# francescovidaich964/TensorNetworkForML

Measured on AMD Instinct MI355X. Metric: sweep-steps/sec, 28x28 MNIST-shaped, bond=20, batch=5000 per GPU, higher is better.
Workload: dtype f32; 1 GPU; c3: N=784 sites, D=2, L=2, bond 20, batch 5000/GPU, softmax+full_cross_ent, trunc=fixed, L2_flag=True; pass = hand-over of one of 4 staged batches + forward + 783-step sweep; global_batch=5000, sweep_steps_per_pass=783, parallelism=dp1, distinct_batches=4

## Files before the change

### tensornetworkforml_amd/csrc/kernels_narrow.hip

```cpp
#include "tnml_internal.h"
#include "jacobi_device.h"
#include "small_gemm_device.h"
#include "wide_pipe_device.h"

namespace tnml {

__device__ inline double wave_sum_f64(double v) {
  v += dpp_f64<0xB1>(v);
  v += dpp_f64<0x4E>(v);
  v += dpp_f64<0x141>(v);
  v += dpp_f64<0x140>(v);
  const double r0 = wave_read_f64(v, 0), r1 = wave_read_f64(v, 16), r2 = wave_read_f64(v, 32), r3 = wave_read_f64(v, 48);
  return (r0 + r1) + (r2 + r3);
}

template <int BUF>
__device__ inline void block_sum3(double &a, double &b, double &c, double *scratch) {
  const int lane = threadIdx.x & 63, wave = threadIdx.x >> 6, nw = blockDim.x >> 6;
  double *s = scratch + BUF * 64;
  a = wave_sum_f64(a); b = wave_sum_f64(b); c = wave_sum_f64(c);
  if (lane == 0) { s[wave] = a; s[16 + wave] = b; s[32 + wave] = c; }
  lds_barrier();
  const int w = lane & 15;
  double ta = w < nw ? s[w] : 0.0, tb = w < nw ? s[16 + w] : 0.0, tc = w < nw ? s[32 + w] : 0.0;
// ... 203 lines not shown
  const int r = D * h, c = D * g * L;
  const bool short_rows = (r <= c);
  const int n = short_rows ? r : c, ne = n + (n & 1), len = short_rows ? c : r;

  unsigned long long t_c0 = 0, t_r0 = 0, t_c1 = 0, t_c2 = 0, t_c2b = 0, t_c2c = 0;
  unsigned long long t_p[5] = {0, 0, 0, 0, 0};
#define TNML_STAMP(i) if (p.stamps && tid == 0) t_p[i] = __builtin_amdgcn_s_memtime()
  if (p.stamps && tid == 0) { t_c0 = __builtin_amdgcn_s_memtime(); t_r0 = __builtin_amdgcn_s_memrealtime(); }
  const int RWz = kD * kD * p.g * p.L;
  const bool fast0 = p.pipe && !p.persist && (size_t)p.z_rows * RWz + (size_t)p.z_rows * h <= (size_t)((float *)k.sOrd - k.fBp) &&
                     Bs <= 8 * NT && p.z_rows * RWz <= 16 * NT && p.z_rows * h <= 4 * NT && h * h <= 2 * NT && g * g <= 2 * NT;
  const PersistLds PL = persist_lds(smem_raw + p.persist_off, p.Mcap);
  float *sRaw = k.fBp;
  if (p.persist) {
    if (tid == 0) {
      const int bad = spin_wait_ge(p.pready, p.pwant, p.abort_flag, 1);
      if (bad == 1) { atomicOr(p.status, 4); __hip_atomic_store(p.abort_flag, 1u, __ATOMIC_RELAXED, __HIP_MEMORY_SCOPE_AGENT); }
      k.sFlag[3] = bad;
    }
    lds_barrier();
    if (k.sFlag[3]) return true;
    if (p.stamps && tid == 0) { p.stamps[20] = (double)(__builtin_amdgcn_s_memtime() - t_c0); p.stamps[28] = (double)(t_r0 & ((1ull << 40) - 1)); p.stamps[29] = (double)(__builtin_amdgcn_s_memrealtime() & ((1ull << 40) - 1)); }
    if (tid < kMetricSlots) k.sTail[tid] = ld_sc1(p.zred + p.zsize + tid);
    for (int e = tid; e < h * h; e += NT) k.dNh[e] = p.Nh ? PL.Nh[e] : 1.0;
    const __amdgpu_buffer_rsrc_t rR = sc1_rsrc(p.prepRaw), rB = sc1_rsrc(p.prepB), rG = sc1_rsrc(p.prepG);
    tn_uvec4 qr[2], qb[2], qg[4];
#pragma unroll
    for (int u = 0; u < 2; ++u) { const int e = 4 * (tid + u * NT); if (e < Bs) { qr[u] = ld_sc1_b128(rR, (unsigned)e * 4u); qb[u] = ld_sc1_b128(rB, (unsigned)e * 4u); } }
#pragma unroll
    for (int u = 0; u < 4; ++u) { const int e = 2 * (tid + u * NT); if (p.l2_flag && e < Bs) qg[u] = ld_sc1_b128(rG, (unsigned)e * 8u); }
#pragma unroll
    for (int u = 0; u < 2; ++u) { const int e = 4 * (tid + u * NT); if (e < Bs) { *reinterpret_cast<tn_uvec4 *>(sRaw + e) = qr[u]; *reinterpret_cast<tn_uvec4 *>(k.fB + e) = qb[u]; } }
#pragma unroll
    for (int u = 0; u < 4; ++u) { const int e = 2 * (tid + u * NT); if (p.l2_flag && e < Bs) *reinterpret_cast<tn_uvec4 *>(k.dG + e) = qg[u]; }
  }
  float *sZ = k.fBp, *sZc = sZ + (size_t)p.z_rows * RWz;
  if (fast0) {
    const int zr = p.z_rows, nz = p.z_first ? 0 : zr * RWz, nzc = p.z_first ? 0 : zr * h;
    const float *zc = p.zcore.base;
    float4 rz[4], rb[2];
    double2 rg[4];
    float rc[4];
    double rnh[2], rng[2];
#pragma unroll
    for (int u = 0; u < 4; ++u) { const int e = 4 * (tid + u * NT); rz[u] = e < nz ? *reinterpret_cast<const float4 *>(p.zred + e) : make_float4(0.f, 0.f, 0.f, 0.f); }
#pragma unroll
    for (int u = 0; u < 2; ++u) { const int e = 4 * (tid + u * NT); rb[u] = (p.prep_ready && e < Bs) ? *reinterpret_cast<const float4 *>(p.prepB + e) : make_float4(0.f, 0.f, 0.f, 0.f); }
#pragma unroll
    for (int u = 0; u < 4; ++u) { const int e = 2 * (tid + u * NT); rg[u] = (p.prep_ready && p.l2_flag && e < Bs) ? *reinterpret_cast<const double2 *>(p.prepG + e) : make_double2(0.0, 0.0); }
    const float inv_h = 1.0f / (float)h;
#pragma unroll
    for (int u = 0; u < 4; ++u) {
      const int e = tid + u * NT, i2 = (int)(((float)e + 0.5f) * inv_h), hh = e - i2 * h;
      rc[u] = e < nzc ? zc[(i2 >> 1) * p.zcore.s_in + (i2 & 1) * p.zcore.s_d + hh * p.zcore.s_out] : 0.f;
    }
#pragma unroll
    for (int u = 0; u < 2; ++u) {
      const int e = tid + u * NT;
      rnh[u] = (p.Nh && e < h * h) ? p.Nh[e] : 1.0;
      rng[u] = (p.Ng && e < g * g) ? p.Ng[e] : 1.0;
    }
#pragma unroll
    for (int u = 0; u < 4; ++u) { const int e = 4 * (tid + u * NT); if (e < nz) *reinterpret_cast<float4 *>(sZ + e) = rz[u]; }
#pragma unroll
    for (int u = 0; u < 2; ++u) { const int e = 4 * (tid + u * NT); if (p.prep_ready && e < Bs) *reinterpret_cast<float4 *>(k.fB + e) = rb[u]; }
#pragma unroll
    for (int u = 0; u < 4; ++u) { const int e = 2 * (tid + u * NT); if (p.prep_ready && p.l2_flag && e < Bs) *reinterpret_cast<double2 *>(k.dG + e) = rg[u]; }
// ... 85 lines not shown
      k.sLab[e] = p.lab.base[h_ * p.lab.s_in + d * p.lab.s_d + s_ * p.lab.s_out + l];
    }
    for (int e = tid; e < s * D * g; e += NT) {
      const int g_ = e % g, q = e / g;
      const int d = q % D, s_ = q / D;
      k.sPl[e] = p.pl.base[s_ * p.pl.s_in + d * p.pl.s_d + g_ * p.pl.s_out];
    }
  } else {
    for (int e = tid; e < Bs; e += NT) k.fB[e] = p.Bdirect[e];
  }
  if (!fast0 && !p.persist) {
    for (int e = tid; e < h * h; e += NT) k.dNh[e] = p.Nh ? p.Nh[e] : 1.0;
    for (int e = tid; e < g * g; e += NT) k.dNg[e] = p.Ng ? p.Ng[e] : 1.0;
  }
  lds_barrier();

  TNML_STAMP(0);
  const int RW = D * D * g * L;
  if (!p.Bdirect && !p.fused && !p.prep_ready && !p.persist) {
    const int QW = D * g;
    small_gemm_f64(L, h * D, QW, s,
                   [&](int l, int i, int kk) { return (double)k.sLab[(i * s + kk) * L + l]; },
                   [&](int l, int kk, int j) { return (double)k.sPl[kk * QW + j]; },
                   [&](int l, int i, int j, double v) { k.fB[(i * QW + j) * L + l] = (float)v; });
  }
  lds_barrier();

  TNML_STAMP(1);
  if (p.l2_flag && !p.fused && !p.prep_ready && !p.persist) {
    mm_lds(1, h, RW, h, k.dNh, 0, 1, h, k.fB, 0, RW, 1, [&](int, int i, int j, double v) { k.dT[i * RW + j] = v; });
    lds_barrier();
    mm_lds(L, Bs / (g * L), g, g, k.dT, 1, g * L, L, k.dNg, 0, g, 1,
           [&](int l, int i, int j, double v) { k.dG[(i * g + j) * L + l] = v; });
    lds_barrier();
  }
  TNML_STAMP(2);
  double sumB = 0.0, sumD = 0.0, l2 = 0.0;
  constexpr int kMaxPer = 8;
  float redv[kMaxPer];
#pragma unroll
  for (int u = 0; u < kMaxPer; ++u) {
    const int e = tid + u * NT;
    redv[u] = (e < Bs && !p.persist && !(p.pipe && !p.z_first)) ? ldred(e) : 0.f;
  }
#pragma unroll
  for (int u = 0; u < kMaxPer; ++u) {
    const int e = tid + u * NT;
    if (e >= Bs) break;
    const double bv = (double)k.fB[e];
    const double raw = p.persist ? (double)sRaw[e] : ((p.pipe && !p.z_first) ? k.dT[e] : (double)redv[u]);
    double wdterm;
    if (p.l2_flag) {
      const double gv = k.dG[e];
      l2 += bv * gv;
      wdterm = 2.0 * (double)p.wd * gv;
    } else {
      wdterm = (double)p.wd * bv;
    }
    const double dv = raw - wdterm;
    if (p.dbg) {
      p.dbg[e] = bv;
      p.dbg[Bs + e] = raw;
      p.dbg[3 * (size_t)Bs + e] = wdterm;
    }
    k.dG[e] = dv;
    sumB += fabs(bv);
// ... 503 lines not shown
           [&](int dk, int h_, int sp, double acc) {
             const float v = (float)acc;
             k.sCb[__mul24(h_ * D + dk, mk) + sp] = v;
             if (p.persist) PL.Ad[__mul24(h_ * D + dk, mk) + sp] = acc;
             st_behind(__mul24(h_, ob_s_h) + dk * ob_s_d + __mul24(sp, ob_s_m), v);
           });
  }
  lds_barrier();
  if (p.persist) {
    if (wave_u == (NT >> 6) - 1) {
      const int ln = tid & 63;
      const __amdgpu_buffer_rsrc_t rP = sc1_rsrc(p.Apub);
      for (int e = ln; e < (r * mk) >> 1; e += 64) st_sc1_b128(rP, (unsigned)e * 16u, pack_d2(PL.Ad[2 * e], PL.Ad[2 * e + 1]));
      for (int e = ln; e < (mk + 1) >> 1; e += 64) {
        const double i0 = k.dSq[ne + 2 * e], i1 = 2 * e + 1 < mk ? k.dSq[ne + 2 * e + 1] : 0.0;
        st_sc1_b128(rP, (unsigned)(r * mk + 2 * e) * 8u, pack_d2(i0 * i0, i1 * i1));
      }
      asm volatile("s_waitcnt vmcnt(0)" ::: "memory");
      if (ln == 0) { unsigned *const aflag = p.aflag; __hip_atomic_store(aflag, (unsigned)p.coretoken, __ATOMIC_RELAXED, __HIP_MEMORY_SCOPE_AGENT); }
    }
  }

  if (p.stamps && tid == 0) t_c2c = __builtin_amdgcn_s_memtime();
  if (Nh_new) {
    if (!short_rows) {
      mm_lds(1, h, DM, h, k.dNh, 0, h, 1, k.sCb, 0, DM, 1, store_T2);
      lds_barrier();
    }
    mm_lds(1, mk, mk, h * D, k.sCb, 0, 1, mk, k.dT2, 0, mk, 1,
           [&](int, int i, int j, double v) {
             Nh_new[__mul24(i, mk) + j] = v;
             if (p.persist) PL.Nh[__mul24(i, mk) + j] = v;
           });
    if (p.persist) {
      lds_barrier();
      const __amdgpu_buffer_rsrc_t rP = sc1_rsrc(p.Apub);
      const int oN = persist_pub_off(r * mk, mk), nn2 = mk * mk;
      for (int e = tid; e < (nn2 + 1) >> 1; e += NT)
        st_sc1_b128(rP, (unsigned)(oN + 2 * e) * 8u, pack_d2(PL.Nh[2 * e], 2 * e + 1 < nn2 ? PL.Nh[2 * e + 1] : 0.0));
    }
  }

  if (p.stamps && tid == 0) {
    const unsigned long long t_c3 = __builtin_amdgcn_s_memtime(), t_r3 = __builtin_amdgcn_s_memrealtime();
    p.stamps[0] = (double)(t_c1 - t_c0); p.stamps[1] = (double)(t_c2 - t_c1); p.stamps[2] = (double)(t_c3 - t_c2);
    p.stamps[3] = (double)(t_r3 - t_r0); p.stamps[4] = (double)sweeps; p.stamps[5] = (double)n;
    p.stamps[50] = (double)round_idx;
    for (int i = 0; i < 5; ++i) p.stamps[9 + i] = (double)(t_p[i] - (i ? t_p[i - 1] : t_c0));
    p.stamps[6] = (double)(t_c2b - t_c2); p.stamps[7] = (double)(t_c2c - t_c2b); p.stamps[8] = (double)(t_c3 - t_c2c);
  }

  if (tid == 0 && p.metrics) {
    const double cnt = (double)ldtail(3);
    const double inv = cnt > 0 ? 1.0 / cnt : 0.0;
    p.metrics[0] = (float)((double)ldtail(0) * inv);
    p.metrics[1] = (float)((double)ldtail(1) * inv / (double)L);
    if (ldtail(2) != 0.f) atomicOr(p.status, 1);
  }
  if (p.persist) {
    asm volatile("s_waitcnt vmcnt(0)" ::: "memory");
    lds_barrier();
    if (tid == 0) { unsigned *const coreflag = p.coreflag; __hip_atomic_store(coreflag, (unsigned)p.coretoken, __ATOMIC_RELAXED, __HIP_MEMORY_SCOPE_AGENT); }
  }
  if (p.done_flag) {
    asm volatile("s_waitcnt vmcnt(0)" ::: "memory");
    __syncthreads();
    if (wave_u == 0) {
      __builtin_amdgcn_fence(__ATOMIC_RELEASE, "agent");
      if (tid == 0) __hip_atomic_store(p.done_flag, p.done_val, __ATOMIC_RELAXED, __HIP_MEMORY_SCOPE_AGENT);
    }
  }
  return false;
}
// ... 84 lines not shown
        for (int e = tid; e < nW; e += NT) {
          const int l = e % L, q = e / L, s_ = q % s, d = r0 + q / s;
          sW[e] = t.lab.base[d * t.lab.s_d + s_ * t.lab.s_out + l];
        }
      }
      for (int e = tid; e < s * DG; e += NT) {
        const int g_ = e % g, q = e / g, d = q % D, s_ = q / D;
        sP[e] = t.pl.base[s_ * t.pl.s_in + d * t.pl.s_d + g_ * t.pl.s_out];
      }
      if (t.l2_flag) for (int e = tid; e < g * g; e += NT) sNg[e] = t.Ng ? t.Ng[e] : 1.0;
      lds_barrier();
      mm_lds(L, nr, DG, s, sW, 1, s * L, L, sP, 0, DG, 1, [&](int l, int row, int col, double v) { oT[(row * DG + col) * L + l] = v; });
      lds_barrier();
      if (t.l2_flag)
        mm_lds(L, nr * D, g, g, oT, 1, g * L, L, sNg, 0, g, 1, [&](int l, int i, int j, double v) { oN[(i * g + j) * L + l] = v; });
      const int nT = nr * DG * L;
      double *Tdst = t.T + (size_t)r0 * DG * L, *Ndst = t.TN + (size_t)r0 * DG * L;
      for (int e = tid; e < nT; e += NT) __hip_atomic_store(Tdst + e, oT[e], __ATOMIC_RELAXED, __HIP_MEMORY_SCOPE_AGENT);
      if (t.l2_flag) {
        lds_barrier();
        for (int e = tid; e < nT; e += NT) __hip_atomic_store(Ndst + e, oN[e], __ATOMIC_RELAXED, __HIP_MEMORY_SCOPE_AGENT);
      }
    }
    asm volatile("s_waitcnt vmcnt(0)" ::: "memory");
    lds_barrier();
    if (tid == 0) __hip_atomic_fetch_add(t.tcnt, 1u, __ATOMIC_RELAXED, __HIP_MEMORY_SCOPE_AGENT);
    return false;
  }
  const bool even_split = RW % nH == 0;
  const int cw = (RW + nH - 1) / nH, c0 = even_split ? hid * cw : min(RW, hid * cw), nc = even_split ? cw : min(RW, c0 + cw) - c0;
  const int cw2 = 2 * cw;
  double *sA = (double *)smem_raw;
  double *sIv = sA + (((size_t)zr * h + 1) & ~(size_t)1);
  double *sNh = sIv + ((h + 1) & ~1);
  double *sS = sNh + (((size_t)h * h + 1) & ~(size_t)1);
  float *sOut = (float *)(sS + persist_helper_ss_doubles(zr, h, cw));
  double *sP2 = (double *)sOut + (size_t)h * cw;
  float *sZf = (float *)(sP2 + (size_t)h * cw);
  float *sAff = sZf + (size_t)zr * cw;
  double *hst = (t.stamps && hid == 0 && tid == 0) ? t.stamps : nullptr;
  double *hst2 = (t.stamps && hid == 0) ? t.stamps : nullptr;
  auto rt = []() { return (double)(__builtin_amdgcn_s_memrealtime() & ((1ull << 40) - 1)); };
  if (tid == 0) { if (hst) hst[22] = rt(); give_up(spin_wait_ge(t.tcnt, (unsigned)nH, t.abort_flag)); if (hst) hst[30] = rt(); }
  lds_barrier();
  if (sBad) return true;
  for (int e = tid; e < zr * nc; e += NT) {
    const int i = e / nc, cc = e - i * nc;
    const size_t src = (size_t)i * RW + c0 + cc;
    sS[i * cw2 + cc] = __hip_atomic_load(t.T + src, __ATOMIC_RELAXED, __HIP_MEMORY_SCOPE_AGENT);
    sS[i * cw2 + cw + cc] = t.l2_flag ? __hip_atomic_load(t.TN + src, __ATOMIC_RELAXED, __HIP_MEMORY_SCOPE_AGENT) : 0.0;
  }
  lds_barrier();
  if (tid == 0) { give_up(spin_wait_ge(t.zready, t.zwant, t.abort_flag)); if (hst) hst[24] = rt(); }
  lds_barrier();
  if (sBad) return true;
  for (int e = tid; e < zr * nc; e += NT) {
    const int i = e / nc, cc = e - i * nc;
    sZf[i * cw + cc] = ld_sc1(t.Z + (size_t)i * RW + c0 + cc);
  }
  lds_barrier();
  if (tid == 0) { give_up(t.awant ? spin_wait_ge(t.aflag, t.awant, t.abort_flag) : 0); if (hst) hst[23] = rt(); }
  lds_barrier();
  if (sBad) return true;
  if (t.awant) {
    const __amdgpu_buffer_rsrc_t rP = sc1_rsrc(t.Apub);
    const int n1 = persist_pub_off(zr * h, h) >> 1, nA = (zr * h) >> 1;
    for (int e = tid; e < n1; e += NT) {
      const tn_uvec4 q = ld_sc1_b128(rP, (unsigned)e * 16u);
      *reinterpret_cast<tn_uvec4 *>(sA + 2 * e) = q;
      if (e < nA) { const dvec2_t a = __builtin_bit_cast(dvec2_t, q); sAff[2 * e] = (float)a[0]; sAff[2 * e + 1] = (float)a[1]; }
    }
  } else if (tid == 0) {
    sA[0] = 1.0; sAff[0] = 1.f; sIv[0] = 1.0; sNh[0] = 1.0;
  }
  lds_barrier();
  if (hst) hst[25] = rt();
  if (nc > 0) {
    mm_lds_f32(h, nc, zr, sAff, 1, h, sZf, cw, 1, [&](int i, int j, float v) { sOut[__mul24(i, cw) + j] = v; });
    const int slot = (((h + 15) >> 4) * ((nc + 15) >> 4)) & ((NT >> 6) - 1);
    mm_lds(1, h, t.l2_flag ? 2 * cw : cw, zr, sA, 0, 1, h, sS, 0, cw2, 1,
           [&](int, int i, int j, double v) {
             if (j < cw) { if (j < nc) sOut[__mul24(h + i, cw) + j] = (float)(v * sIv[i]); }
             else sP2[__mul24(i, cw) + (j - cw)] = v * sIv[i];
           }, false, slot);
  }
  if (t.l2_flag) {
    if (t.awant && (tid >> 6) == (NT >> 6) - 1) {
      const int ln = tid & 63;
      int bad = 0;
      if (ln == 0) { if (hst2) hst2[31] = rt(); bad = spin_wait_ge(t.nflag, t.awant, t.abort_flag); give_up(bad); if (hst2) hst2[21] = rt(); }
      if (!__builtin_amdgcn_readfirstlane(bad)) {
        const __amdgpu_buffer_rsrc_t rP = sc1_rsrc(t.Apub);
        const int oN = persist_pub_off(zr * h, h), nq = (h * h + 1) >> 1;
        for (int e0 = ln; e0 < nq; e0 += 4 * 64) {
          tn_uvec4 q[4];
#pragma unroll
          for (int u = 0; u < 4; ++u) if (e0 + 64 * u < nq) q[u] = ld_sc1_b128(rP, (unsigned)(oN + 2 * (e0 + 64 * u)) * 8u);
#pragma unroll
          for (int u = 0; u < 4; ++u) if (e0 + 64 * u < nq) *reinterpret_cast<tn_uvec4 *>(sNh + 2 * (e0 + 64 * u)) = q[u];
        }
      }
    }
  }
  lds_barrier();
  if (t.l2_flag && sBad) return true;
  st_sc1_rows(t.prepRaw, sOut, h, cw, RW, c0, nc);
  st_sc1_rows(t.prepB, sOut + (size_t)h * cw, h, cw, RW, c0, nc);
  if (t.l2_flag) {
    if (nc > 0) {
      mm_lds(1, h, nc, h, sNh, 0, 1, h, sP2, 0, cw, 1, [&](int, int i, int j, double v) { sS[__mul24(i, cw) + j] = v; });
    }
    lds_barrier();
    st_sc1_rows(t.prepG, sS, h, cw, RW, c0, nc);
  }
  if (hst) hst[26] = rt();
  asm volatile("s_waitcnt vmcnt(0)" ::: "memory");
  lds_barrier();
  if (tid == 0) __hip_atomic_fetch_add(t.pcnt, 1u, __ATOMIC_RELAXED, __HIP_MEMORY_SCOPE_AGENT);
  if (hst) hst[27] = rt();
  return false;
}

template <class Shape>
struct HelperArgs : PersistHelperParams {
  static constexpr int zr = Shape::zr, s = Shape::s, g = Shape::g, L = Shape::L, h = Shape::h;
  __device__ __forceinline__ explicit HelperArgs(const PersistHelperParams &q) : PersistHelperParams(q) {}
};
__device__ __forceinline__ int rec_shape(const PersistStep *rec) { return *(const __attribute__((address_space(4))) int *)&rec->shape; }

template <class Shape>
__global__ __launch_bounds__(kNarrowThreads) void sweep_persist_kernel(const PersistStep *__restrict__ steps_g, int n_steps, int nH) {
  extern __shared__ __attribute__((aligned(16))) unsigned char smem_raw[];
  const int blk = blockIdx.x;
  if (blk == 0) {
#pragma nounroll
    for (int k = 0; k < n_steps; ++k) {
      if constexpr (Shape::id != 0) {
        if (rec_shape(&steps_g[k]) == Shape::id) {
          if (narrow_body(PersistArgs<Shape>(&steps_g[k].n), smem_raw)) break;
          continue;
        }
      }
      if (narrow_body(PersistArgs<DynShape>(&steps_g[k].n), smem_raw)) break;
    }
  } else if (blk <= nH) {
#pragma nounroll
    for (int ph = 0; ph < 2 * n_steps; ++ph) {
// ... 115 lines not shown
```

### tensornetworkforml_amd/csrc/san/hip_stub.cpp

```cpp
#include <hip/hip_runtime.h>
#include <rccl/rccl.h>
#include <sys/mman.h>
#include <cstdarg>
#include <cstdio>
#include <cstdlib>
#include <cstring>
#include <map>
#include <string>
#include <vector>
#include <cxxabi.h>
#include "../tnml_internal.h"
#include "../wide_pipe_device.h"
#include "../grad_chain_device.h"

using namespace tnml;

namespace san {
static char *g_base = nullptr;
static size_t g_used = 0;
static constexpr size_t kArena = (size_t)1 << 38, kGap = (size_t)1 << 20;
static std::map<uintptr_t, size_t> &alloc_map() { static auto *m = new std::map<uintptr_t, size_t>; return *m; }
static std::map<const void *, std::string> &kernel_map() { static auto *m = new std::map<const void *, std::string>; return *m; }
static std::map<std::string, long> &launch_map() { static auto *m = new std::map<std::string, long>; return *m; }
#define g_alloc alloc_map()
// ... 370 lines not shown
static std::string dp(const void *p) {
  if (!p) return "0";
  if (!in_arena(p)) return "host";
  char b[24];
  snprintf(b, sizeof b, "@%zx", (size_t)((const char *)p - g_base));
  return b;
}
static void *new_handle(int kind) { static long next[2]; long *h = (long *)malloc(sizeof(long)); *h = next[kind]++; return h; }
static long id(const void *h) { return h ? *(const long *)h : -1; }
#define I(f) tr(" " #f "=%lld", (long long)p.f);
#define R(f) tr(" " #f "=%.17g", (double)p.f);
#define P(f) tr(" " #f "=%s", dp(p.f).c_str());
#define V(f) tr(" " #f "=[%s %d %d %d %d %d]", dp(p.f.base).c_str(), p.f.n_in, p.f.n_out, p.f.s_in, p.f.s_d, p.f.s_out);
static void tr_struct(const NarrowParams &p) {
  I(L) I(D) I(h) I(g) I(s) I(m) I(bsize) I(l2_flag) R(lr) R(wd) R(inv_b_global) P(red) V(lab) V(pl) P(Nh) P(Ng) P(Bnew)
  P(out_behind) I(ob_s_h) I(ob_s_d) I(ob_s_m) P(out_ahead) I(oa_s_m) I(oa_s_d) I(oa_s_g) P(Nh_new) P(metrics) P(dbg) P(stamps)
  P(counters) P(Bdirect) I(stop_after_update) I(fused) I(prep_ready) P(slabs) I(nslabs) I(slab_stride) I(nred) P(red_out) P(prepB)
  P(prepG) P(sync) R(trunc_thr) I(left_dir) P(m_out) R(chol_thr) R(svd_stop2) P(status) I(wait_count) I(pipe) I(z_first) I(z_rows)
  I(zsize) P(zred) V(zcore) P(flag) I(token) I(persist) I(write_ahead) I(persist_off) I(Mcap) P(prepRaw) P(pready) I(pwant) P(Apub)
  P(aflag) P(coreflag) I(coretoken) P(zpoll_flag) I(zpoll_want) P(done_flag) I(done_val) P(abort_flag)
}
static void tr_struct(const WideParams &p) {
  I(b) I(b_pad) I(L) I(h) I(g) I(hp) I(gp) I(do_f) I(do_ext) I(first_ext) I(act_fn) I(loss_fn) R(T) P(x_km1) P(x_k) P(x_kp1) P(Hprev)
  P(Hcur) P(Gprev) P(Gcur) P(Bprev) V(ext_core) P(y) P(f) P(slabs) I(slab_stride) I(bsize) P(stamps)
}
static void tr_struct(const WidePipeParams &p) {
  I(b) I(b_pad) I(L) I(hj) I(gj) I(gn) I(hprev) I(first) I(do_ext) I(first_ext) I(do_f) I(wait_flag) I(do_z) I(act_fn) I(loss_fn) R(T)
  P(x_jm1) P(x_j) P(x_jp1) P(x_jp2) P(Eprev) P(Ecur) V(ext_core) P(Gj) P(Gn) P(Bnew) P(y) P(f) I(zsize) I(slab_stride) P(slabs) P(gslabs)
  P(zred) P(gcnt) P(tcnt) I(nwide) I(gsz) I(ngroups) I(one_level) I(wg0) I(tiles_per_wg) I(ntiles) P(flag) I(token) P(status) I(persist)
  P(coreflag) I(corewant) P(zready) I(zpublish) P(abort_flag) P(stamps)
}
static void tr_struct(const PersistHelperParams &p) {
  I(zr) I(s) I(g) I(L) I(h) I(l2_flag) P(W) V(lab) V(pl) P(Ng) P(T) P(TN) P(Z) P(prepRaw) P(prepB) P(prepG) P(Apub) P(flag) I(want)
  P(aflag) P(nflag) I(awant) P(zready) I(zwant) P(tcnt) P(pcnt) P(abort_flag) P(status) P(stamps)
}
static void tr_struct(const PersistStep &p) { tr(" n:"); tr_struct(p.n); tr(" w:"); tr_struct(p.w); tr(" t:"); tr_struct(p.t); tr(" shape=%d", p.shape); }
static void tr_struct(const PrepParams &p) { V(lab) V(pl) P(Nh) P(Ng) I(h) I(g) I(s) I(L) I(l2_flag) P(prepB) P(prepG) I(nparts) }
static void tr_struct(const MeetParams &p) { P(Lenv) P(Renv) P(x) P(core) P(f) I(b) I(b_pad) I(ml) I(mr) I(D) I(L) I(rows_per_chunk) }
static void tr_struct(const InputGradParams &p) {
  P(bond) P(cores) P(labcore) P(X) P(cot) P(stack) P(g) P(cf) I(core_stride) I(b) I(b_pad) I(x_bpad) I(N) I(D) I(L) I(l_pos) I(cap) I(mb)
}
static void tr_struct(const CoreGradParams &p) {
  P(tab) P(cores) P(labcore) P(X) P(cot) P(stackP) P(stackQ) P(G) P(cf) I(core_stride) I(b) I(b_pad) I(x_bpad) I(N) I(D) I(L) I(l_pos) I(cap)
  I(mb) I(first)
}
static void tr_struct(const InputGradScaledParams &p) { tr_struct(p.base); P(estack) }
static void tr_struct(const CoreGradScaledParams &p) { tr_struct(p.base); P(estack) }
static void tr_struct(const ScaledPredParams &p) { P(bond) P(cores) P(labcore) P(X) P(mant) P(expo) P(f) I(core_stride) I(b) I(b_pad) I(N) I(D) I(L) I(l_pos) I(mb) }
static void tr_struct(const LossCotParams &p) { P(f) P(y) P(cot) I(L) I(b) I(b_pad) I(f_bpad) I(act_fn) I(loss_fn) R(T) }
static void tr_struct(const OptimStepParams &p) {
  P(tab) P(cores) P(labcore) P(G) P(s0) P(s1) I(core_stride) I(N) I(D) I(L) I(l_pos) I(kind) I(clip) R(lr) R(wd) R(mu) R(beta1) R(beta2) R(eps)
  R(corr1) R(corr2)
}
static void tr_struct(const InputGradPixels &p) { P(g) P(data) P(idx) P(out) I(b) I(N) I(D) }
static void tr_struct(const BigExtArgs &p) { P(Eprev) P(x_km1) P(x_k) V(A) I(b_pad) P(Ecur) P(Pk) }
static void tr_struct(const ChainSite &p) { I(core_off) I(is_label) I(n_in) I(n_out) I(s_in) I(s_d) I(s_out) I(x_site) I(env_out_off) }
static void tr_struct(const NormChainSite &p) { I(core_off) I(n_in) I(n_out) I(s_in) I(s_d) I(s_out) I(env_out_off) }
#undef I
#undef R
#undef P
#undef V
template <class S> static void tr_rows(const char *what, const S *rows, int n) {
  for (int i = 0; i < n; ++i) { tr("  %s %d:", what, i); tr_struct(rows[i]); tr("\n"); }
}
static void tr_launch(const std::string &name, dim3 g, dim3 b, size_t shm, hipStream_t st, void **args) {
  const size_t lp = name.find('('), rp = name.rfind(')');
  tr("launch %s grid=%u,%u,%u block=%u,%u,%u lds=%zu stream=s%ld", name.substr(0, lp).c_str(), g.x, g.y, g.z, b.x, b.y, b.z, shm, id(st));
// ... 325 lines not shown
```

### tensornetworkforml_amd/csrc/tnml_api.hip

```cpp
#include <rccl/rccl.h>

#include <algorithm>
#include <climits>
#include <cmath>
#include <cstdarg>
#include <cstdio>
#include <cstring>
#include <cstdlib>
#include <initializer_list>
#include <memory>
#include <utility>

#include "tnml_internal.h"
#include "small_gemm_device.h"
#include "wide_pipe_device.h"
#include "grad_chain_device.h"

using namespace tnml;

static thread_local std::string g_err;

static int fail(int code, const char *fmt, ...) {
  char buf[1024];
  va_list ap;
// ... 2118 lines not shown
    n.stamps = (c->stamps && k == n_steps / 2) ? c->dbg + 4 * c->bmax + kDbgSigma + 5 : nullptr;
    n.pipe = 1; n.persist = 1; n.z_first = (k == 0);
    fill_wide_pipe(c, ps.w, sc, k);
    WidePipeParams &wp = ps.w;
    const int zr = k == 0 ? 1 : wp.hprev * D;
    if (zr > 64) return give_up();
    n.z_rows = zr; n.zsize = zr * D * D * g * L;
    n.zred = zr2[k & 1]; n.red = n.zred;
    n.prepB = c->prepB; n.prepG = c->prepG; n.prepRaw = c->prepRaw;
    n.pready = c->pst_cnt + (size_t)k * 32 + 21; n.pwant = (unsigned)nH;
    n.flag = fl + 0; n.token = (unsigned)k + 1;
    n.Apub = c->Apub;
    n.aflag = fl + 5; n.coreflag = fl + 3; n.coretoken = (unsigned)k + 1; n.abort_flag = fl + 4;
    n.Mcap = Mcap;
    if (!persist_record_ok(n)) return give_up();
    lds_narrow = std::max(lds_narrow, nlds);
    wp.do_ext = k >= 1; wp.do_f = 1; wp.wait_flag = 1;
    wp.do_z = (k + 1 <= N - 2);
    set_pipe_tiles(wp, tpw);
    wp.wg0 = 1 + nH; wp.persist = 1; wp.flag = fl + 0; wp.token = (unsigned)k + 1;
    wp.coreflag = fl + 3; wp.corewant = (unsigned)k; wp.zready = fl + 2; wp.zpublish = (unsigned)k + 2; wp.abort_flag = fl + 4;
    wp.zred = zr2[(k + 1) & 1];
    wp.gcnt = c->pst_cnt + (size_t)k * 32; wp.tcnt = wp.gcnt + 16;
    wp.stamps = n.stamps;
    if (!wide_pipe_fits(c, wp)) return give_up();
    pipe_try_one_level(wp);
    lds_wide = std::max(lds_wide, wide_pipe_lds_bytes(wp));
    PersistHelperParams &t = ps.t;
    t.zr = zr; t.s = s; t.g = g; t.L = L; t.h = h; t.l2_flag = n.l2_flag;
    t.W = k == 0 ? nullptr : c->Bnew;
    t.lab = n.lab; t.pl = n.pl; t.Ng = n.Ng;
    t.T = c->Tbuf[k & 1]; t.TN = c->TNbuf[k & 1]; t.Z = zr2[k & 1];
    t.prepRaw = c->prepRaw; t.prepB = c->prepB; t.prepG = c->prepG; t.Apub = c->Apub;
    t.flag = fl + 0; t.want = (unsigned)k; t.aflag = fl + 5; t.nflag = fl + 3; t.awant = (unsigned)k; t.zready = fl + 2; t.zwant = (unsigned)k + 1;
    t.tcnt = c->pst_cnt + (size_t)k * 32 + 20; t.pcnt = c->pst_cnt + (size_t)k * 32 + 21;
    t.abort_flag = fl + 4; t.status = c->status; t.stamps = n.stamps;
    lds_help = std::max(lds_help, persist_helper_lds_bytes(zr, s, g, L, h, nH));
    if ((size_t)zr * D * D * g * L + kMetricSlots > (size_t)c->zstride) return give_up();
    advance_frame(c, q, m);
    if (!c->stamps || k <= n_steps / 2) note_last_step(c, q);
    add_step_work(c, q, bytes, flops);
  }
  const size_t lds = c->persist_mode >= 2 ? lds_narrow + pbytes : std::max(std::max(lds_narrow + pbytes, lds_wide), lds_help);
  if (lds > kLdsMax || lds_wide > kLdsMax || lds_help > kLdsMax) return give_up();
  const int persist_off = (int)((lds - pbytes) & ~(size_t)15);
  for (int k = 0; k < n_steps; ++k) st[k].n.persist_off = persist_off;
  int shape = 0, n_fixed = 0;
  if (c->shape_kernels && c->persist_mode < 2)
    for (int k = 0; k < n_steps; ++k) {
      const NarrowParams &n = st[k].n;
      const PersistHelperParams &t = st[k].t;
      const int id = persist_step_shape(n.h, n.g, n.s, n.m, n.L, n.z_rows, n.bsize, nH);
      if (!id || (shape && id != shape) || n.D != kD) continue;
      if (persist_step_shape(t.h, t.g, t.s, n.m, t.L, t.zr, n.bsize, nH) != id) continue;
      shape = id; st[k].shape = id; ++n_fixed;
    }
  HIP_TRY(hipMemcpyAsync(c->pst_dev, st, (size_t)(n_steps + 1) * sizeof(PersistStep), hipMemcpyHostToDevice, c->stream));
  HIP_TRY(hipEventRecord(c->pst_ev[buf], c->stream));
  c->pst_cur ^= 1;
  HIP_TRY(hipMemsetAsync(c->pst_flags, 0, 8 * sizeof(unsigned), c->stream));
  HIP_TRY(hipMemsetAsync(c->pst_cnt, 0, (size_t)(n_steps + 1) * 32 * sizeof(unsigned), c->stream));
  if (c->persist_mode >= 2) {
    HIP_TRY(hipEventRecord(c->ev_p0, c->stream));
    HIP_TRY(hipStreamWaitEvent(c->stream2, c->ev_p0, 0));
    HIP_TRY(hipStreamWaitEvent(c->stream3, c->ev_p0, 0));
    launch_sweep_persist_split(c->pst_dev, n_steps, nH, nwide, lds, lds_help, lds_wide, c->stream, c->stream2, c->stream3);
    HIP_TRY(hipGetLastError());
// ... 833 lines not shown
```

### tensornetworkforml_amd/csrc/wide_pipe_device.h

```cpp
#pragma once
#include "tnml_internal.h"
#include "act_device.h"
#include "jacobi_device.h"

namespace tnml {

typedef float fvec4 __attribute__((ext_vector_type(4)));
constexpr int kPipeThreads = 1024;
constexpr int kPTSP = kTS + 1;
constexpr int kPipeGroupMax = 16;

__host__ __device__ inline int upm(int x, int m) { return (x + m - 1) / m * m; }

__device__ inline void st_sc1(float *p, float v) { __hip_atomic_store(p, v, __ATOMIC_RELAXED, __HIP_MEMORY_SCOPE_AGENT); }
__device__ inline float ld_sc1(const float *p) { return __hip_atomic_load(p, __ATOMIC_RELAXED, __HIP_MEMORY_SCOPE_AGENT); }

struct WidePipeParams {
  int b, b_pad, L;
  int hj, gj;
  int gn;
  int hprev;
  int first;
  int do_ext;
  int first_ext;
// ... 89 lines not shown
  w.sQn = q; q += (p.do_z ? d.J3 * kPTSP : 0);
  w.sFp = q; q += (p.do_f ? (size_t)(d.IP / 16) * p.L * kTS : 0);
  w.sMet = q; q += 4 * kTS;
  w.floats = (size_t)(q - base);
  return w;
}
inline size_t wide_pipe_lds_bytes(const WidePipeParams &p) {
  const WidePipeDims d = wide_pipe_dims(p);
  alignas(16) static float origin[4];
  return wide_pipe_carve(origin, p, d).floats * sizeof(float) + 16;
}
constexpr int kPipeMaxZT = 4;
inline int wide_pipe_ztiles(const WidePipeParams &p) {
  const WidePipeDims d = wide_pipe_dims(p);
  return p.L * (d.I3 / 16) * (d.J3 / 16);
}
void launch_step_pipe(const NarrowParams &p, const WidePipeParams &w, size_t lds_bytes, hipStream_t st);
void launch_step_pipe_update(const NarrowParams &p, const WidePipeParams &w, size_t lds_bytes, hipStream_t st);

struct PersistHelperParams {
  int zr, s, g, L, h;
  int l2_flag;
  const float *W;
  CoreView lab, pl;
  const double *Ng;
  double *T, *TN;
  const float *Z;
  float *prepRaw, *prepB;
  double *prepG;
  const double *Apub;
  const unsigned *flag;
  unsigned want;
  const unsigned *aflag;
  const unsigned *nflag;
  unsigned awant;
  const unsigned *zready;
  unsigned zwant;
  unsigned *tcnt, *pcnt;
  unsigned *abort_flag;
  int *status;
  double *stamps;
};
struct PersistStep { NarrowParams n; WidePipeParams w; PersistHelperParams t; int shape; int pad_; };
constexpr int kPersistHelpers = 8;
struct PersistShape { int H, L; };
constexpr PersistShape kPersistShapes[] = {{10, 2}, {20, 2}};
constexpr int kNumPersistShapes = (int)(sizeof(kPersistShapes) / sizeof(kPersistShapes[0]));
template <int H, int LBL, int ID>
struct FixedShape {
  static constexpr int id = ID;
  static constexpr int h = H, g = H, s = H, m = H, L = LBL, bsize = H * kD * kD * H * LBL, zr = kD * H, nH = kPersistHelpers;
  static_assert(H >= 1 && H <= 64 && kD * H <= 64 && ((kD * H) & 1) == 0 && bsize <= 8192, "beyond the in-LDS persistent step");
  template <class R> __device__ __forceinline__ void load_shape(const R *) {}
  static constexpr bool fits(int h_, int g_, int s_, int m_, int L_, int z_rows_, int bsize_, int nH_) {
    return h_ == h && g_ == g && s_ == s && m_ == m && L_ == L && z_rows_ == zr && bsize_ == bsize && nH_ == nH;
  }
};
template <int I = 0>
constexpr int persist_step_shape(int h, int g, int s, int m, int L, int z_rows, int bsize, int nH) {
  if constexpr (I < kNumPersistShapes) {
    return FixedShape<kPersistShapes[I].H, kPersistShapes[I].L, I + 1>::fits(h, g, s, m, L, z_rows, bsize, nH)
               ? I + 1 : persist_step_shape<I + 1>(h, g, s, m, L, z_rows, bsize, nH);
  } else {
    return 0;
  }
}
__host__ __device__ inline int persist_pub_off(int na, int h) { return ((na + 1) & ~1) + ((h + 1) & ~1); }
__host__ __device__ inline size_t persist_pub_doubles(int na, int h) { return (size_t)persist_pub_off(na, h) + (((size_t)h * h + 1) & ~(size_t)1); }
__host__ __device__ inline size_t persist_helper_ss_doubles(int zr, int h, int cw) {
  const size_t a = 2 * (size_t)zr * cw, b = (size_t)h * cw;
  return ((a > b ? a : b) + 1) & ~(size_t)1;
}
inline size_t persist_helper_lds_bytes(int zr, int s, int g, int L, int h, int nH) {
  const size_t DG = (size_t)kD * g, RW = kD * DG * L;
  const size_t per = ((size_t)zr * kD + nH - 1) / nH, cw = (RW + nH - 1) / nH;
  const size_t p1 = (((per * s * L + 3) & ~(size_t)3) + (((size_t)s * DG + 3) & ~(size_t)3)) * sizeof(float) +
                    ((((size_t)g * g + 1) & ~(size_t)1) + 2 * per * DG * L) * sizeof(double);
  const size_t p2 = (persist_pub_doubles(zr * h, h) + persist_helper_ss_doubles(zr, h, (int)cw) + 2 * (size_t)h * cw) * sizeof(double) +
                    ((size_t)zr * cw + (size_t)zr * h) * sizeof(float);
  return (p1 > p2 ? p1 : p2) + 64;
}
bool launch_sweep_persist(const PersistStep *steps_dev, int n_steps, int n_helpers, int grid, size_t lds_bytes, hipStream_t st, int shape);
void launch_sweep_persist_split(const PersistStep *steps_dev, int n_steps, int n_helpers, int n_wide, size_t lds_update, size_t lds_helper,
                                size_t lds_wide, hipStream_t st_update, hipStream_t st_helper, hipStream_t st_wide);


template <int PERSIST>
struct WidePipeArgs : WidePipeParams {
  __device__ __forceinline__ WidePipeArgs(const WidePipeParams &q) : WidePipeParams(q) {}
  static constexpr int persist = PERSIST;
};
template <class WP>
__device__ __forceinline__ bool wide_pipe_block(const WP &p, float *smem) {
  const WidePipeDims dm = wide_pipe_dims(p);
  const WidePipeSmem w = wide_pipe_carve(smem, p, dm);
  int tid_step = threadIdx.x;
  if (p.persist) {
    asm volatile("" : "+v"(tid_step));
    __builtin_assume(tid_step >= 0 && tid_step < kPipeThreads);
  }
  const int tid = tid_step, NT = kPipeThreads;
  const int lane = tid & 63, NWV = NT / 64;
  const int wave = __builtin_amdgcn_readfirstlane(tid >> 6);
  const int r = lane & 15, q = lane >> 4;
  const int L = p.L, hj = p.hj, gj = p.gj, gn = p.gn, hprev = p.hprev;
  const int nI = dm.nI, nJ = kD * gj;
  constexpr int ST = kTS / 16;
  const int wg = (int)blockIdx.x - p.wg0;
  const int IT3 = dm.I3 / 16, JT3 = dm.J3 / 16, QW = kD * gn;
  constexpr int kMaxZT = kPipeMaxZT;
  fvec4 zacc[kMaxZT];
// ... 344 lines not shown
```

Before: 22110 sweep-steps/s.

## Apply Nh to L2 prep in update block instead of helpers

Helpers now store the un-normalised P2 product as prepG without waiting for the freshly published Nh. The update block loads it into dT and multiplies by its local Nh before the step, so Nh no longer needs publishing to global memory. This removes a flag wait and a global Nh round-trip from the helper path. In exchange it adds an h×RW matmul plus a barrier to the update block's serial critical path.

```diff
diff --git a/tensornetworkforml_amd/csrc/kernels_narrow.hip b/tensornetworkforml_amd/csrc/kernels_narrow.hip
--- a/tensornetworkforml_amd/csrc/kernels_narrow.hip
+++ b/tensornetworkforml_amd/csrc/kernels_narrow.hip
@@ -259,7 +259,7 @@
 #pragma unroll
     for (int u = 0; u < 2; ++u) { const int e = 4 * (tid + u * NT); if (e < Bs) { *reinterpret_cast<tn_uvec4 *>(sRaw + e) = qr[u]; *reinterpret_cast<tn_uvec4 *>(k.fB + e) = qb[u]; } }
 #pragma unroll
-    for (int u = 0; u < 4; ++u) { const int e = 2 * (tid + u * NT); if (p.l2_flag && e < Bs) *reinterpret_cast<tn_uvec4 *>(k.dG + e) = qg[u]; }
+    for (int u = 0; u < 4; ++u) { const int e = 2 * (tid + u * NT); if (p.l2_flag && e < Bs) *reinterpret_cast<tn_uvec4 *>(k.dT + e) = qg[u]; }
   }
   float *sZ = k.fBp, *sZc = sZ + (size_t)p.z_rows * RWz;
   if (fast0) {
@@ -411,6 +411,10 @@
     lds_barrier();
     mm_lds(L, Bs / (g * L), g, g, k.dT, 1, g * L, L, k.dNg, 0, g, 1,
            [&](int l, int i, int j, double v) { k.dG[(i * g + j) * L + l] = v; });
+    lds_barrier();
+  }
+  if (p.l2_flag && p.persist) {
+    mm_lds(1, h, RW, h, k.dNh, 0, 1, h, k.dT, 0, RW, 1, [&](int, int i, int j, double v) { k.dG[__mul24(i, RW) + j] = v; });
     lds_barrier();
   }
   TNML_STAMP(2);
@@ -980,13 +984,6 @@
              Nh_new[__mul24(i, mk) + j] = v;
              if (p.persist) PL.Nh[__mul24(i, mk) + j] = v;
            });
-    if (p.persist) {
-      lds_barrier();
-      const __amdgpu_buffer_rsrc_t rP = sc1_rsrc(p.Apub);
-      const int oN = persist_pub_off(r * mk, mk), nn2 = mk * mk;
-      for (int e = tid; e < (nn2 + 1) >> 1; e += NT)
-        st_sc1_b128(rP, (unsigned)(oN + 2 * e) * 8u, pack_d2(PL.Nh[2 * e], 2 * e + 1 < nn2 ? PL.Nh[2 * e + 1] : 0.0));
-    }
   }
 
   if (p.stamps && tid == 0) {
@@ -1137,14 +1134,12 @@
   const int cw2 = 2 * cw;
   double *sA = (double *)smem_raw;
   double *sIv = sA + (((size_t)zr * h + 1) & ~(size_t)1);
-  double *sNh = sIv + ((h + 1) & ~1);
-  double *sS = sNh + (((size_t)h * h + 1) & ~(size_t)1);
-  float *sOut = (float *)(sS + persist_helper_ss_doubles(zr, h, cw));
+  double *sS = sIv + ((h + 1) & ~1);
+  float *sOut = (float *)(sS + persist_helper_ss_doubles(zr, cw));
   double *sP2 = (double *)sOut + (size_t)h * cw;
   float *sZf = (float *)(sP2 + (size_t)h * cw);
   float *sAff = sZf + (size_t)zr * cw;
   double *hst = (t.stamps && hid == 0 && tid == 0) ? t.stamps : nullptr;
-  double *hst2 = (t.stamps && hid == 0) ? t.stamps : nullptr;
   auto rt = []() { return (double)(__builtin_amdgcn_s_memrealtime() & ((1ull << 40) - 1)); };
   if (tid == 0) { if (hst) hst[22] = rt(); give_up(spin_wait_ge(t.tcnt, (unsigned)nH, t.abort_flag)); if (hst) hst[30] = rt(); }
   lds_barrier();
@@ -1169,14 +1164,14 @@
   if (sBad) return true;
   if (t.awant) {
     const __amdgpu_buffer_rsrc_t rP = sc1_rsrc(t.Apub);
-    const int n1 = persist_pub_off(zr * h, h) >> 1, nA = (zr * h) >> 1;
+    const int n1 = persist_pub_doubles(zr * h, h) >> 1, nA = (zr * h) >> 1;
     for (int e = tid; e < n1; e += NT) {
       const tn_uvec4 q = ld_sc1_b128(rP, (unsigned)e * 16u);
       *reinterpret_cast<tn_uvec4 *>(sA + 2 * e) = q;
       if (e < nA) { const dvec2_t a = __builtin_bit_cast(dvec2_t, q); sAff[2 * e] = (float)a[0]; sAff[2 * e + 1] = (float)a[1]; }
     }
   } else if (tid == 0) {
-    sA[0] = 1.0; sAff[0] = 1.f; sIv[0] = 1.0; sNh[0] = 1.0;
+    sA[0] = 1.0; sAff[0] = 1.f; sIv[0] = 1.0;
   }
   lds_barrier();
   if (hst) hst[25] = rt();
@@ -1189,35 +1184,11 @@
              else sP2[__mul24(i, cw) + (j - cw)] = v * sIv[i];
            }, false, slot);
   }
-  if (t.l2_flag) {
-    if (t.awant && (tid >> 6) == (NT >> 6) - 1) {
-      const int ln = tid & 63;
-      int bad = 0;
-      if (ln == 0) { if (hst2) hst2[31] = rt(); bad = spin_wait_ge(t.nflag, t.awant, t.abort_flag); give_up(bad); if (hst2) hst2[21] = rt(); }
-      if (!__builtin_amdgcn_readfirstlane(bad)) {
-        const __amdgpu_buffer_rsrc_t rP = sc1_rsrc(t.Apub);
-        const int oN = persist_pub_off(zr * h, h), nq = (h * h + 1) >> 1;
-        for (int e0 = ln; e0 < nq; e0 += 4 * 64) {
-          tn_uvec4 q[4];
-#pragma unroll
-          for (int u = 0; u < 4; ++u) if (e0 + 64 * u < nq) q[u] = ld_sc1_b128(rP, (unsigned)(oN + 2 * (e0 + 64 * u)) * 8u);
-#pragma unroll
-          for (int u = 0; u < 4; ++u) if (e0 + 64 * u < nq) *reinterpret_cast<tn_uvec4 *>(sNh + 2 * (e0 + 64 * u)) = q[u];
-        }
-      }
-    }
-  }
-  lds_barrier();
-  if (t.l2_flag && sBad) return true;
+  lds_barrier();
+  if (hst) hst[31] = rt();
   st_sc1_rows(t.prepRaw, sOut, h, cw, RW, c0, nc);
   st_sc1_rows(t.prepB, sOut + (size_t)h * cw, h, cw, RW, c0, nc);
-  if (t.l2_flag) {
-    if (nc > 0) {
-      mm_lds(1, h, nc, h, sNh, 0, 1, h, sP2, 0, cw, 1, [&](int, int i, int j, double v) { sS[__mul24(i, cw) + j] = v; });
-    }
-    lds_barrier();
-    st_sc1_rows(t.prepG, sS, h, cw, RW, c0, nc);
-  }
+  if (t.l2_flag) st_sc1_rows(t.prepG, sP2, h, cw, RW, c0, nc);
   if (hst) hst[26] = rt();
   asm volatile("s_waitcnt vmcnt(0)" ::: "memory");
   lds_barrier();
diff --git a/tensornetworkforml_amd/csrc/san/hip_stub.cpp b/tensornetworkforml_amd/csrc/san/hip_stub.cpp
--- a/tensornetworkforml_amd/csrc/san/hip_stub.cpp
+++ b/tensornetworkforml_amd/csrc/san/hip_stub.cpp
@@ -426,7 +426,7 @@
 }
 static void tr_struct(const PersistHelperParams &p) {
   I(zr) I(s) I(g) I(L) I(h) I(l2_flag) P(W) V(lab) V(pl) P(Ng) P(T) P(TN) P(Z) P(prepRaw) P(prepB) P(prepG) P(Apub) P(flag) I(want)
-  P(aflag) P(nflag) I(awant) P(zready) I(zwant) P(tcnt) P(pcnt) P(abort_flag) P(status) P(stamps)
+  P(aflag) I(awant) P(zready) I(zwant) P(tcnt) P(pcnt) P(abort_flag) P(status) P(stamps)
 }
 static void tr_struct(const PersistStep &p) { tr(" n:"); tr_struct(p.n); tr(" w:"); tr_struct(p.w); tr(" t:"); tr_struct(p.t); tr(" shape=%d", p.shape); }
 static void tr_struct(const PrepParams &p) { V(lab) V(pl) P(Nh) P(Ng) I(h) I(g) I(s) I(L) I(l2_flag) P(prepB) P(prepG) I(nparts) }
diff --git a/tensornetworkforml_amd/csrc/tnml_api.hip b/tensornetworkforml_amd/csrc/tnml_api.hip
--- a/tensornetworkforml_amd/csrc/tnml_api.hip
+++ b/tensornetworkforml_amd/csrc/tnml_api.hip
@@ -2174,7 +2174,7 @@
     t.lab = n.lab; t.pl = n.pl; t.Ng = n.Ng;
     t.T = c->Tbuf[k & 1]; t.TN = c->TNbuf[k & 1]; t.Z = zr2[k & 1];
     t.prepRaw = c->prepRaw; t.prepB = c->prepB; t.prepG = c->prepG; t.Apub = c->Apub;
-    t.flag = fl + 0; t.want = (unsigned)k; t.aflag = fl + 5; t.nflag = fl + 3; t.awant = (unsigned)k; t.zready = fl + 2; t.zwant = (unsigned)k + 1;
+    t.flag = fl + 0; t.want = (unsigned)k; t.aflag = fl + 5; t.awant = (unsigned)k; t.zready = fl + 2; t.zwant = (unsigned)k + 1;
     t.tcnt = c->pst_cnt + (size_t)k * 32 + 20; t.pcnt = c->pst_cnt + (size_t)k * 32 + 21;
     t.abort_flag = fl + 4; t.status = c->status; t.stamps = n.stamps;
     lds_help = std::max(lds_help, persist_helper_lds_bytes(zr, s, g, L, h, nH));
diff --git a/tensornetworkforml_amd/csrc/wide_pipe_device.h b/tensornetworkforml_amd/csrc/wide_pipe_device.h
--- a/tensornetworkforml_amd/csrc/wide_pipe_device.h
+++ b/tensornetworkforml_amd/csrc/wide_pipe_device.h
@@ -145,7 +145,6 @@
   const unsigned *flag;
   unsigned want;
   const unsigned *aflag;
-  const unsigned *nflag;
   unsigned awant;
   const unsigned *zready;
   unsigned zwant;
@@ -178,18 +177,14 @@
     return 0;
   }
 }
-__host__ __device__ inline int persist_pub_off(int na, int h) { return ((na + 1) & ~1) + ((h + 1) & ~1); }
-__host__ __device__ inline size_t persist_pub_doubles(int na, int h) { return (size_t)persist_pub_off(na, h) + (((size_t)h * h + 1) & ~(size_t)1); }
-__host__ __device__ inline size_t persist_helper_ss_doubles(int zr, int h, int cw) {
-  const size_t a = 2 * (size_t)zr * cw, b = (size_t)h * cw;
-  return ((a > b ? a : b) + 1) & ~(size_t)1;
-}
+__host__ __device__ inline int persist_pub_doubles(int na, int h) { return ((na + 1) & ~1) + ((h + 1) & ~1); }
+__host__ __device__ inline size_t persist_helper_ss_doubles(int zr, int cw) { return 2 * (size_t)zr * cw; }
 inline size_t persist_helper_lds_bytes(int zr, int s, int g, int L, int h, int nH) {
   const size_t DG = (size_t)kD * g, RW = kD * DG * L;
   const size_t per = ((size_t)zr * kD + nH - 1) / nH, cw = (RW + nH - 1) / nH;
   const size_t p1 = (((per * s * L + 3) & ~(size_t)3) + (((size_t)s * DG + 3) & ~(size_t)3)) * sizeof(float) +
                     ((((size_t)g * g + 1) & ~(size_t)1) + 2 * per * DG * L) * sizeof(double);
-  const size_t p2 = (persist_pub_doubles(zr * h, h) + persist_helper_ss_doubles(zr, h, (int)cw) + 2 * (size_t)h * cw) * sizeof(double) +
+  const size_t p2 = ((size_t)persist_pub_doubles(zr * h, h) + persist_helper_ss_doubles(zr, cw) + 2 * (size_t)h * cw) * sizeof(double) +
                     ((size_t)zr * cw + (size_t)zr * h) * sizeof(float);
   return (p1 > p2 ? p1 : p2) + 64;
 }
```

Measured after the change: 22340 sweep-steps/s (median of 6 runs). 1.0% higher.
